# cvxgrp/qcqp

Hardware: AMD Instinct MI355X
Metric: restarts x coord-sweeps / sec (improve COORD_DESCENT phase-2 sweeps, 2n^2 flops each; whole step timed) (higher is better)
Workload: dtype f64

## Files before the change

### qcqp_amd/csrc/cd_life.hip

```cpp
#include "cd_life.h"

#include <cstdio>
#include <cstdlib>

#include "onevar.h"
#include "cd_phase1_sep.h"
#include "cd_chain.h"
#include "cd_roles.h"

namespace qcqpmi {
namespace {

constexpr int L2_WD = 1 << 21;
enum { L2_ABORT = 3 };

__device__ __attribute__((always_inline)) inline RqOwn l2_own(int NB, int CS, int m, int NMW) {
    RqOwn o;
    const int rest = NB - CS;
    o.NB = NB;
    if (m < 0) { o.first = rest; o.stride = 1; o.nu = CS; }
    else { o.first = m; o.stride = NMW; o.nu = m < rest ? (rest - m + NMW - 1) / NMW : 0; }
    return o;
}

constexpr int L2_SHARED_DOUBLES = 8 + 8 + 16 + 8;
constexpr int L2_YBMAX = 18;
constexpr int L2_YU = 6;
constexpr int L2_KCL = 4;
constexpr int l2_tile_doubles(int nmw, int csu, int lr, int kcl = 1, int maxc = 1) {
    return 2 * nmw * 256 + 256 + 256 + 2 * 256 + 2 * 48 + 4 * 256 + csu * 256 + 16 + 8 + 16 * 4 + 8 * 5 + 64 * 10 + 16 * 3 + 8 * 5 + 32 +
           (lr ? L2_YBMAX * 256 + 2 * 256 : 0) +
           2 * (maxc + 1) * 16 * kcl + 2 * 8 * kcl + (kcl > 1 ? 16 : 0);
}
#define L2_LDS_VIEW(tile_) \
    extern __shared__ double smem[]; \
    int *ctl = (int *)smem; \
    int *simdof = (int *)(smem + 8); \
    int *p1cols = (int *)(smem + 16); \
    int *jn = (int *)(smem + 32); \
    double *sp = smem + L2_SHARED_DOUBLES + (tile_) * l2_tile_doubles(NMW, CSU, LRV, KCLV, MAXC); \
    double *part2 = sp; sp += 2 * NMW * 256; \
    double *fixp = sp; sp += 256; \
    double *gtile = sp; sp += 256; \
    double *DU2 = sp; sp += 2 * 256; \
    double *sc2 = sp; sp += 2 * 48; \
    double *ring = sp; sp += 4 * 256; \
    double *cshare = sp; sp += CSU * 256; \
// ... 153 lines not shown
                else L2_LDA(arP + 2 * U, so2 + ((U < nu) ? NMW * 2048 * U : 0), vlane)
            }
        }
        acc = acc + acc1;
        if (i >= 2) {
            const long long tw0 = prof_on ? (long long)__builtin_amdgcn_s_memtime() : 0;
            for (;;) {
                const rq_i4 s4 = rq_sync_read(sy);
                if (s4[RQ_STOP]) { stop = true; break; }
                if (s4[RQ_CONS] >= (int)i - 1) break;
                if (++spins > L2_WD) { stop = true; rq_sync_write(sy, L2_ABORT, 1, lane); rq_sync_write(sy, RQ_STOP, 1, lane); break; }
                __builtin_amdgcn_s_sleep(1);
            }
            if (stop) break;
            spins = 0;
            if (prof_on) pw_cons += (long long)__builtin_amdgcn_s_memtime() - tw0;
        }
        {
            double *part = part2 + (int)(i & 1) * NMW * 256 + m * 256;
    #pragma unroll
            for (int v = 0; v < 4; v++) part[v * 64 + (lane & 15) * 4 + (lane >> 4)] = acc[v];
        }
        rq_sync_write(sy, RQ_PARTS + m, (int)i + 1, lane);
        row = row2;
    }
    if (prof_on && lane == 0) {
        atomicAdd(pprof + 9, (unsigned long long)pw_commit);
        atomicAdd(pprof + 10, (unsigned long long)pw_cons);
    }
    #undef L2_LDA
}


template <int NMW>
__device__ __attribute__((noinline)) void l2_mfma_lr_role(int m_in, int t_in) {
    constexpr int MAXC = 1;
    constexpr int KCLV = 1;
    constexpr int CSU = 1;
    constexpr int LRV = 1;
    constexpr int YU = L2_YU;
    const int tile = l2_uni(t_in);
    L2_LDS_VIEW(tile)
    (void)clsb;
    (void)fixp; (void)gtile; (void)DU2; (void)sc2; (void)cshare; (void)slk; (void)TC; (void)of0; (void)ovis; (void)oacc; (void)oswp; (void)sid; (void)snew;
    (void)sfin; (void)ost; (void)ctl; (void)cst; (void)sseed; (void)sfirst; (void)p1key; (void)p1upd; (void)p1fin; (void)p1sw; (void)p1st; (void)gatep; (void)simdof; (void)p1cols; (void)jn;
    const int lane = threadIdx.x & 63;
    const int m = l2_uni(m_in);
    const double *pG = l2_uni(par->Gpack), *pU = l2_uni(par->Upack);
    const int NB = l2_uni(par->NB), RB = l2_uni(par->RB);
    const int nu = (RB > m) ? (RB - m + NMW - 1) / NMW : 0;
    const int64_t gmax = (int64_t)1 << 40;
    const __amdgpu_buffer_rsrc_t grsrc = __builtin_amdgcn_make_buffer_rsrc(const_cast<double *>(pG), 0, NB * RB * 2048, 0x00020000);
    const __amdgpu_buffer_rsrc_t ursrc = __builtin_amdgcn_make_buffer_rsrc(const_cast<double *>(pU), 0, NB * RB * 2048, 0x00020000);
    const unsigned vlane = (unsigned)lane * 16u;
    typedef unsigned rq_u4 __attribute__((ext_vector_type(4)));
    #define L2_LDF(dst, rs, soff) { const rq_u4 t0_ = __builtin_amdgcn_raw_buffer_load_b128(rs, vlane, (soff), 0);           \
                                    const rq_u4 t1_ = __builtin_amdgcn_raw_buffer_load_b128(rs, vlane + 1024u, (soff), 0);   \
                                    (dst)[0] = __builtin_bit_cast(v2d_, t0_); (dst)[1] = __builtin_bit_cast(v2d_, t1_); }
    typedef __attribute__((address_space(3))) double rq_lds_d;
    typedef __attribute__((address_space(3))) const double rq_lds_cd;
    const int yoff = (lane >> 4) * 16 + (lane & 15);
    rq_lds_d *ybase = (rq_lds_d *)(ytile + yoff);
    rq_lds_cd *rbase = (rq_lds_cd *)(ring + lane);
    rq_lds_cd *pbase = (rq_lds_cd *)(pend + lane);
    asm volatile("" : "+v"(ybase), "+v"(rbase), "+v"(pbase));
    v4d_ y[YU];
    #pragma unroll
    for (int u = 0; u < YU; u++)
    #pragma unroll
        for (int v = 0; v < 4; v++) y[u][v] = (u < nu) ? ybase[(16 * (m + NMW * u) + 4 * v) * 16] : 0.0;
    auto save_y = [&]() {
    #pragma unroll
        for (int u = 0; u < YU; u++)
            if (u < nu) {
    #pragma unroll
                for (int v = 0; v < 4; v++) ybase[(16 * (m + NMW * u) + 4 * v) * 16] = y[u][v];
            }
    };
    int row = 0, spins = 0;
    int yrow = 0;
    int64_t iy = 0;
    for (int64_t i = 0; i < gmax; i++) {
        const int row2 = (row + 1 == NB) ? 0 : row + 1;
        const int ub = row >= 3 ? row - 3 : row - 3 + NB;
        v2d_ aU[YU][2], aG[YU][2];
    #pragma unroll
        for (int u = 0; u < YU; u++)
            if (u < nu) {
                L2_LDF(aU[u], ursrc, (ub * RB + m + NMW * u) * 2048)
                L2_LDF(aG[u], grsrc, (row * RB + m + NMW * u) * 2048)
            }
        bool stop = false;
        if (i >= 3) {
            for (;;) {
                const rq_i4 s4 = rq_sync_read(sy);
                if (s4[RQ_STOP]) { stop = true; break; }
                if (s4[RQ_COMMIT] >= (int)i - 2) break;
                if (++spins > L2_WD) { stop = true; rq_sync_write(sy, L2_ABORT, 1, lane); rq_sync_write(sy, RQ_STOP, 1, lane); break; }
                __builtin_amdgcn_s_sleep(1);
            }
            if (stop) break;
            spins = 0;
        }
        if (i >= 1) {
            if (row == 1) save_y();
            rq_lds_cd *src = (i >= 3) ? rbase + (int)((i - 3) & 3) * 256 : pbase + (int)(i - 1) * 256;
            double bd[4];
    #pragma unroll
            for (int q = 0; q < 4; q++) bd[q] = src[q * 64];
    #pragma unroll
            for (int v = 0; v < 4; v++)
    #pragma unroll
                for (int u = 0; u < YU; u++)
                    if (u < nu) y[u] = __builtin_amdgcn_mfma_f64_16x16x4f64(aU[u][v >> 1][v & 1], bd[v], y[u], 0, 0, 0);
            yrow = row; iy = i;
        }
        v4d_ acc = {0.0, 0.0, 0.0, 0.0}, acc1 = acc;
    #pragma unroll
        for (int u = 0; u < YU; u++)
            if (u < nu) {
                acc = __builtin_amdgcn_mfma_f64_16x16x4f64(aG[u][0][0], y[u][0], acc, 0, 0, 0);
                acc1 = __builtin_amdgcn_mfma_f64_16x16x4f64(aG[u][0][1], y[u][1], acc1, 0, 0, 0);
                acc = __builtin_amdgcn_mfma_f64_16x16x4f64(aG[u][1][0], y[u][2], acc, 0, 0, 0);
                acc1 = __builtin_amdgcn_mfma_f64_16x16x4f64(aG[u][1][1], y[u][3], acc1, 0, 0, 0);
            }
        acc = acc + acc1;
        if (i >= 2) {
            for (;;) {
                const rq_i4 s4 = rq_sync_read(sy);
                if (s4[RQ_STOP]) { stop = true; break; }
                if (s4[RQ_CONS] >= (int)i - 1) break;
                if (++spins > L2_WD) { stop = true; rq_sync_write(sy, L2_ABORT, 1, lane); rq_sync_write(sy, RQ_STOP, 1, lane); break; }
                __builtin_amdgcn_s_sleep(1);
            }
            if (stop) break;
            spins = 0;
        }
        {
            double *part = part2 + (int)(i & 1) * NMW * 256 + m * 256;
    #pragma unroll
            for (int v = 0; v < 4; v++) part[v * 64 + (lane & 15) * 4 + (lane >> 4)] = acc[v];
        }
        rq_sync_write(sy, RQ_PARTS + m, (int)i + 1, lane);
        row = row2;
    }
    if (yrow == NB - 1 && iy >= 3) {
        v2d_ aU[YU][2];
    #pragma unroll
        for (int u = 0; u < YU; u++)
            if (u < nu) L2_LDF(aU[u], ursrc, ((NB - 3) * RB + m + NMW * u) * 2048)
        rq_lds_cd *src = rbase + (int)((iy - 2) & 3) * 256;
        double bd[4];
    #pragma unroll
        for (int q = 0; q < 4; q++) bd[q] = src[q * 64];
    #pragma unroll
        for (int v = 0; v < 4; v++)
    #pragma unroll
            for (int u = 0; u < YU; u++)
                if (u < nu) y[u] = __builtin_amdgcn_mfma_f64_16x16x4f64(aU[u][v >> 1][v & 1], bd[v], y[u], 0, 0, 0);
        save_y();
    } else if (yrow == 0) {
        save_y();
    }
    #undef L2_LDF
}

template <int NMW, int CS, int KIND, int TILES, int LR>
__device__ __attribute__((noinline)) void l2_chain_role(int t_in) {
    constexpr bool MULTI = KIND == L2_KIND_GENK || KIND == L2_KIND_LINK;
    constexpr int BK = KIND == L2_KIND_GENK ? L2_KIND_GEN : KIND == L2_KIND_LINK ? L2_KIND_LIN : KIND;
    constexpr int MAXC = MULTI ? 2 : 1;
    constexpr int KCLV = MULTI ? L2_KCL : 1;
    constexpr int CSU = CS > 0 ? CS : 1;
    constexpr int LRV = LR;
    static_assert(!LR || CS == 0, "factored objective: the chain has no share of the contraction");
    static_assert(!MULTI || (TILES == 1 && !LR), "multi-class kinds: one tile per workgroup, no objective factor");
    constexpr bool PRE = BK == L2_KIND_LIN || BK == L2_KIND_SGN;
    const int tile = TILES > 1 ? l2_uni(t_in) : 0;
    L2_LDS_VIEW(tile)
    (void)ytile; (void)pend; (void)clsb;
    (void)slk; (void)snew; (void)p1key; (void)p1upd; (void)p1fin; (void)p1sw; (void)p1st; (void)gatep; (void)simdof; (void)p1cols; (void)jn;
    const int lane = threadIdx.x & 63, r = lane >> 2, gq = lane & 3;
    GLB const double *Apk = glb(l2_uni(par->Apack));
    GLB const double *Apk2 = glb(l2_uni(par->Apack2));
    GLB const double *Dpk = glb(l2_uni(par->Dpack));
    GLB const double *Spk = glb(l2_uni(par->Spack));
    GLB double *Xg = glb(l2_uni(par->Xg));
    GLB const int *pnext = glb(l2_uni(par->next));
    GLB const int *clsg = glb(l2_uni(par->cls));
    unsigned long long *pprof = l2_uni(par->prof);
    const int pRtotal = l2_uni(par->Rtotal);
    const int NB = l2_uni(par->NB), KS = l2_uni(par->KS), nlast = l2_uni(par->nlast);
    struct { int64_t n; double r0; } P = {(int64_t)l2_uni(par->n), l2_uni(par->r0)};
    struct { double tol, fbound; int64_t num_iters; } a = {l2_uni(par->tol), l2_uni(par->fbound), (int64_t)l2_uni(par->num_iters)};
    const int64_t gmax = (int64_t)1 << 40;
    __builtin_amdgcn_s_setprio(3);
    const int Un = TC.n[r], Uslow = TC.slow[r];
    const double Ul0 = TC.lo[r], Uh0 = TC.hi[r], Ul1 = TC.lo[16 + r], Uh1 = TC.hi[16 + r];
    const bool two = Un >= 2;
    const double thr = two ? 1e-7 * (Ul1 - Uh0) : 0.0;
    const double syma = two ? Ul1 : 0.0, symb = two ? Uh1 : Uh0;
    const double gmid = two ? 0.5 * (Uh0 + Ul1) : QM_INF;
    const double linL = Ul0, linH = two ? Uh1 : Uh0;
    auto lin_tl = [&](double l0_, double h0_, double l1_, double h1_, bool two_) {
        const double lL = l0_, lH = two_ ? h1_ : h0_;
        const double w0 = h0_ - l0_, w1 = two_ ? h1_ - l1_ : w0;
        const double wmin = w0 < w1 ? w0 : w1;
        const double hh = fabs(lL) > fabs(lH) ? fabs(lL) : fabs(lH);
        const double scale = a.fbound * (hh * hh > 1.0 ? hh * hh : 1.0);
        return (wmin > 0.0) ? 0.5e-12 * scale / wmin : QM_INF;
    };
    double tl = 0.0;
    if ((BK == L2_KIND_LIN || BK == L2_KIND_SGN) && !MULTI) tl = lin_tl(Ul0, Uh0, Ul1, Uh1, two);
    const double omid = (BK == L2_KIND_SGN) ? 0.5 * (linL + linH) : 0.0;
    struct { int upd_counter, visits, accepted, sweeps, status; bool conv; } S;
    S.upd_counter = (int)cst[0 * 64 + lane]; S.visits = (int)cst[1 * 64 + lane]; S.accepted = (int)cst[2 * 64 + lane];
    S.sweeps = (int)cst[3 * 64 + lane]; S.conv = cst[4 * 64 + lane] != 0; S.status = (int)cst[5 * 64 + lane];
    double fpart = __longlong_as_double(cst[6 * 64 + lane]);
    bool frz = (cst[7 * 64 + lane] & 1) != 0, done = (cst[7 * 64 + lane] & 2) != 0, pre = PRE && (cst[7 * 64 + lane] & 4) != 0;
    bool ld = LR && (cst[7 * 64 + lane] & 8) != 0;
    double facc = __longlong_as_double(cst[8 * 64 + lane]);
    const bool occupied = sid[r] >= 0;
    const RqOwn cown = l2_own(NB, CS, -1, NMW);
    v2d_ arC[2 * CSU];
    double afix[4] = {0.0, 0.0, 0.0, 0.0}, afix2[4] = {0.0, 0.0, 0.0, 0.0};
    v4d_ carry = {0.0, 0.0, 0.0, 0.0};
    double xon[4], d4[4], s3 = 0.0;
    {
    #pragma unroll
        for (int e = 0; e < 4; e++) d4[e] = Dpk[lane + 64 * e];
        if (lane < 48) s3 = Spk[lane];
    #pragma unroll
        for (int v = 0; v < 4; v++) xon[v] = Xg[(4 * v + gq) * 16 + r];
    #pragma unroll
        for (int e = 0; e < 4; e++) DU2[lane + 64 * e] = d4[e];
        if (lane < 48) sc2[lane] = s3;
        if (MULTI && lane < 16) clsb[lane] = (lane < l2_uni(par->n)) ? clsg[lane] : 0;
        v4d_ c0 = {0.0, 0.0, 0.0, 0.0}, c1 = {0.0, 0.0, 0.0, 0.0};
        const int bl2 = NB - 2, bl1 = NB - 1;
        double f0a[4], f0b[4], f1b[4], x2[4], x1[4];
    #pragma unroll
        for (int u = 0; u < 4; u++) {
            f0a[u] = Apk[((int64_t)0 * KS + 4 * bl2 + u) * 64 + lane];
            f0b[u] = Apk[((int64_t)0 * KS + 4 * bl1 + u) * 64 + lane];
            f1b[u] = Apk[((int64_t)1 * KS + 4 * bl1 + u) * 64 + lane];
            x2[u] = LR ? pend[u * 64 + lane] : Xg[(4 * bl2 + u) * 64 + lane];
            x1[u] = LR ? pend[256 + u * 64 + lane] : Xg[(4 * bl1 + u) * 64 + lane];
        }
    #pragma unroll
        for (int u = 0; u < 4; u++) c0 = __builtin_amdgcn_mfma_f64_16x16x4f64(f0a[u], x2[u], c0, 0, 0, 0);
    #pragma unroll
        for (int u = 0; u < 4; u++) {
            c0 = __builtin_amdgcn_mfma_f64_16x16x4f64(f0b[u], x1[u], c0, 0, 0, 0);
            c1 = __builtin_amdgcn_mfma_f64_16x16x4f64(f1b[u], x1[u], c1, 0, 0, 0);
        }
        carry = c1;
        if (CS > 0) {
            rq_load_A<CSU>(arC, Apk2, KS, cown, lane, 0);
            double bqC[4 * CSU];
    #pragma unroll
            for (int U = 0; U < CSU; U++) {
                const int bb = rq_block(cown, U);
    #pragma unroll
                for (int q = 0; q < 4; q++) bqC[4 * U + q] = Xg[(4 * bb + q) * 64 + lane];
            }
    #pragma unroll
            for (int U = 0; U < CSU; U++)
    #pragma unroll
                for (int q = 0; q < 4; q++) cshare[U * 256 + q * 64 + lane] = bqC[4 * U + q];
            c0 = rq_product<CSU>(arC, bqC, Apk2, KS, cown, lane, rq_slot(cown, bl1), rq_slot(cown, bl2), 1, c0);
        }
    #pragma unroll
        for (int v = 0; v < 4; v++) fixp[v * 64 + (lane & 15) * 4 + (lane >> 4)] = c0[v];
    }
    const double tolv = a.tol;
    int b = 0, spins = 0;
    bool wdog = false;
    const bool prof_on = pprof != nullptr;
    long long pw_part = 0, pt_sum = 0, pt_steps = 0, pt_end = 0, pt_fix = 0, pt_req = 0, ptl = 0;
    if (prof_on) { ptl = (long long)__builtin_amdgcn_s_memtime(); if (lane == 0) atomicAdd(pprof + 18, (unsigned long long)(ptl - *(long long *)(ctl + 6))); }
    int pn_int = 0, pn_gen = 0;
#define L2_TICK(acc) if (prof_on) { const long long now_ = (long long)__builtin_amdgcn_s_memtime(); acc += now_ - ptl; ptl = now_; }
    int64_t last_g = 0;
    for (int64_t g = 0; g < gmax; g++) {
        last_g = g;
        const int bn = (b + 1 == NB) ? 0 : b + 1, bn2 = (bn + 1 == NB) ? 0 : bn + 1;
        const int bprev = (b == 0) ? NB - 1 : b - 1;
        const int cur = (int)(g & 1);
        const double *DU = DU2 + cur * 256, *hqb = sc2 + cur * 48, *rtb = sc2 + cur * 48 + 16, *dgb = sc2 + cur * 48 + 32;
        const double *part = part2 + cur * NMW * 256;
        double *rb = ring + (int)(g & 3) * 256;
        const int ncol = (b == NB - 1) ? nlast : 16;
        double xo[4];
    #pragma unroll
        for (int v = 0; v < 4; v++) xo[v] = xon[v];
    #pragma unroll
        for (int e = 0; e < 4; e++) d4[e] = Dpk[(int64_t)bn * 256 + lane + 64 * e];
        if (lane < 48) s3 = Spk[(int64_t)bn * 48 + lane];
        int c3 = 0;
        if (MULTI && lane < 16) c3 = (16 * bn + lane < (int)P.n) ? clsg[16 * bn + lane] : 0;
    #pragma unroll
        for (int v = 0; v < 4; v++) xon[v] = Xg[(16 * (int64_t)bn + 4 * v + gq) * 16 + r];
        {
            GLB const double *ap = Apk + ((int64_t)bn * KS + 4 * b) * 64 + lane;
            GLB const double *ap2 = Apk + ((int64_t)bn2 * KS + 4 * b) * 64 + lane;
    #pragma unroll
            for (int u = 0; u < 4; u++) { afix[u] = ap[u * 64]; afix2[u] = ap2[u * 64]; }
        }
        const long long tw0 = prof_on ? (long long)__builtin_amdgcn_s_memtime() : 0;
        for (;;) {
            const rq_i4 p4 = rq_sync_read(sy + RQ_PARTS);
            int lo4 = p4[0] < p4[1] ? p4[0] : p4[1];
            const int lo2 = p4[2] < p4[3] ? p4[2] : p4[3];
            lo4 = lo4 < lo2 ? lo4 : lo2;
            if (NMW > 4) {
                const rq_i4 q4 = rq_sync_read(sy + RQ_PARTS + 4);
                const int l1 = q4[0] < q4[1] ? q4[0] : q4[1], l2 = q4[2] < q4[3] ? q4[2] : q4[3];
                lo4 = lo4 < l1 ? lo4 : l1;
                lo4 = lo4 < l2 ? lo4 : l2;
            }
            if (lo4 >= (int)g + 1) break;
            if (++spins > L2_WD) { wdog = true; break; }
            __builtin_amdgcn_s_sleep(1);
        }
        if (wdog) { rq_sync_write(sy, L2_ABORT, 1, lane); break; }
        spins = 0;
        if (prof_on) { pt_req += tw0 - ptl; ptl = (long long)__builtin_amdgcn_s_memtime(); pw_part += ptl - tw0; pn_int++; }
        double gb[4], xn[4], rto[4], t2o[4], hq4[4];
    #pragma unroll
        for (int v = 0; v < 4; v++) {
            double s = fixp[v * 64 + lane];
    #pragma unroll
            for (int w = 0; w < NMW; w++) s += part[w * 256 + v * 64 + lane];
            hq4[v] = hqb[4 * v + gq];
            s += hq4[v];
            gb[v] = s;
            gtile[(4 * v + gq) * 16 + r] = s;
        }
        rq_sync_write(sy, RQ_CONS, (int)g + 1, lane);
    #pragma unroll
// ... 167 lines not shown
                    DrawKey dk{dseed, dfirst + (uint64_t)sid[r], (uint32_t)i, (uint32_t)(G.sweeps - 1) | 0x80000000u, 0u};
                    double xnew = xi;
                    int got;
                    if (BK == L2_KIND_LIN && cslow == 0 && C.n > 0 && fabs(gc) > ctl_) {
                        xnew = (gc > 0.0) ? clinL : clinH;
                        got = G.conv ? 0 : 1;
                    } else {
                        got = G.conv ? 0 : onevar_minimise<MAXC>(t2g, t1, t0, C, dk, &xnew);
                    }
                    bool moved;
                    double delta;
                    const bool wasconv = G.conv;
                    chain_commit<MAXC>(G, got, xnew, xi, t2g, t1, t0, a.tol, P.n, moved, delta);
                    if (!wasconv) fa = moved ? 0.0 : fa + xi * (gc + hq);
                    if (moved) {
                        rb[c * 16 + r] = xnew;
                        for (int c2 = c + 1; c2 < 16; c2++) gtile[c2 * 16 + r] += DU[c * 16 + c2] * delta;
                    }
                }
                S.upd_counter = (int)G.upd_counter; S.visits = (int)G.visits; S.accepted = (int)G.accepted; S.conv = G.conv; S.status = G.status;
                fpart = (gq == 0) ? G.fcur : 0.0;
                facc = (gq == 0) ? fa : 0.0;
                if (S.conv) done = true;
#pragma unroll
                for (int v = 0; v < 4; v++) xn[v] = rb[(4 * v + gq) * 16 + r];
                if (LR) {
#pragma unroll
                    for (int v = 0; v < 4; v++) rb[(4 * v + gq) * 16 + r] = xn[v] - xo[v];
                }
            }
        }
    #pragma unroll
        for (int v = 0; v < 4; v++) Xg[(16 * (int64_t)b + 4 * v + gq) * 16 + r] = xn[v];
        rq_sync_write(sy, RQ_COMMIT, (int)g + 1, lane);
        L2_TICK(pt_end)
        if (b == NB - 1) {
            if (ld) { ld = false; if (!frz) S.conv = false; }
            else if (frz) { frz = false; done = true; }
            if (PRE && pre) {
                const double f0s = rq_quad_sum(facc) + P.r0;
                fpart = (gq == 0) ? f0s : 0.0;
                facc = 0.0; pre = false; S.conv = false;
            }
        }
        const unsigned long long livem = __builtin_amdgcn_ballot_w64(!S.conv || frz || pre || ld);
        if (TILES == 1) {
            if (livem == 0ull) break;
            if (b == NB - 1) {
                const bool fin = !occupied || done;
                const unsigned long long finm = __builtin_amdgcn_ballot_w64(fin);
                if (finm == ~0ull) break;
                if (finm != 0ull) {
                    const bool more = glb_load_int(pnext) < pRtotal;
                    if (more) break;
                }
            }
        } else if (b == NB - 1) {
            const unsigned long long finm = __builtin_amdgcn_ballot_w64(!occupied || done);
            const int mine = (livem != 0ull ? 1 : 0) | (finm == ~0ull ? 2 : 0) | (finm != 0ull ? 4 : 0);
            const int tag = ((int)(g / NB) + 1) << 8;
            rq_lds_int *jw = (rq_lds_int *)jn;
            int verdict = 0;
            if (tile == 1) rq_sync_write(jw, 1, tag | mine, lane);
            for (;;) {
                int w = *(volatile rq_lds_int *)(jw + (tile == 1 ? 0 : 1));
                asm volatile("" ::: "memory");
                w = __builtin_amdgcn_readfirstlane(w);
                if ((w & ~0xff) == tag) { verdict = w & 0xff; break; }
                if (++spins > L2_WD) { wdog = true; break; }
                __builtin_amdgcn_s_sleep(1);
            }
            if (wdog) { rq_sync_write(sy, L2_ABORT, 1, lane); break; }
            spins = 0;
            if (tile == 0) {
                const int both = mine | verdict, all = mine & verdict;
                bool stop = !(both & 1) || (all & 2);
                if (!stop && (both & 4)) stop = glb_load_int(pnext) < pRtotal;
                rq_sync_write(jw, 0, tag | (stop ? 1 : 0), lane);
                verdict = stop ? 1 : 0;
            }
            if (verdict & 1) break;
        }
        {
            v4d_ acc = carry, acc2 = {0.0, 0.0, 0.0, 0.0};
            double xb4[4];
    #pragma unroll
            for (int u = 0; u < 4; u++) xb4[u] = rb[u * 64 + lane];
    #pragma unroll
            for (int u = 0; u < 4; u++) {
                acc = __builtin_amdgcn_mfma_f64_16x16x4f64(afix[u], xb4[u], acc, 0, 0, 0);
                acc2 = __builtin_amdgcn_mfma_f64_16x16x4f64(afix2[u], xb4[u], acc2, 0, 0, 0);
            }
            carry = acc2;
            if (CS > 0) {
                const int us = rq_slot(cown, b);
                if (us >= 0) {
    #pragma unroll
                    for (int q = 0; q < 4; q++) cshare[us * 256 + q * 64 + lane] = xb4[q];
                }
                double bqC[4 * CSU];
    #pragma unroll
                for (int U = 0; U < CSU; U++)
    #pragma unroll
                    for (int q = 0; q < 4; q++) bqC[4 * U + q] = cshare[U * 256 + q * 64 + lane];
                acc = rq_product<CSU>(arC, bqC, Apk2, KS, cown, lane, us, rq_slot(cown, bprev), bn2, acc);
            }
    #pragma unroll
            for (int v = 0; v < 4; v++) fixp[v * 64 + (lane & 15) * 4 + (lane >> 4)] = acc[v];
        }
        {
            const int nx = (int)((g + 1) & 1);
    #pragma unroll
            for (int e = 0; e < 4; e++) DU2[nx * 256 + lane + 64 * e] = d4[e];
            if (lane < 48) sc2[nx * 48 + lane] = s3;
            if (MULTI && lane < 16) clsb[nx * 16 + lane] = c3;
        }
        L2_TICK(pt_fix)
        b = bn;
    }
#undef L2_TICK
    if (LR) {
        const int g1 = (int)((last_g - 1) & 3), g0 = (int)(last_g & 3);
        double p1v[4], p0v[4];
#pragma unroll
        for (int u = 0; u < 4; u++) { p1v[u] = ring[g1 * 256 + u * 64 + lane]; p0v[u] = ring[g0 * 256 + u * 64 + lane]; }
#pragma unroll
        for (int u = 0; u < 4; u++) { pend[u * 64 + lane] = p1v[u]; pend[256 + u * 64 + lane] = p0v[u]; }
    }
    rq_sync_write(sy, RQ_STOP, 1, lane);
    if (prof_on && lane == 0) {
        atomicAdd(pprof + 13, (unsigned long long)pt_sum);
        atomicAdd(pprof + 14, (unsigned long long)pt_steps);
        atomicAdd(pprof + 15, (unsigned long long)pt_end);
        atomicAdd(pprof + 19, (unsigned long long)pt_req);
        *(long long *)(ctl + 8) = (long long)__builtin_amdgcn_s_memtime();
        atomicAdd(pprof + 7, (unsigned long long)pt_fix);
        atomicAdd(pprof + 8, (unsigned long long)pw_part);
        atomicAdd(pprof + 11, (unsigned long long)pn_int);
        atomicAdd(pprof + 12, (unsigned long long)pn_gen);
    }
    {
        cst[0 * 64 + lane] = S.upd_counter; cst[1 * 64 + lane] = S.visits; cst[2 * 64 + lane] = S.accepted;
        cst[3 * 64 + lane] = S.sweeps; cst[4 * 64 + lane] = S.conv ? 1 : 0; cst[5 * 64 + lane] = S.status;
        cst[6 * 64 + lane] = __double_as_longlong(fpart);
        cst[7 * 64 + lane] = (frz ? 1 : 0) | (done ? 2 : 0) | (pre ? 4 : 0) | (ld ? 8 : 0);
        cst[8 * 64 + lane] = __double_as_longlong(facc);
        const double ftot = rq_quad_sum(facc) + P.r0;
        const bool fin = occupied && done;
        if (gq == 0) {
            sfin[r] = fin ? 1 : 0;
            if (fin) { ovis[r] = S.visits; oacc[r] = S.accepted; oswp[r] = S.sweeps; ost[r] = S.status; of0[r] = ftot; }
        }
    }
    __builtin_amdgcn_s_setprio(0);
}

template <int NMW, int CS, int KIND, int TILES, int LR>
__global__ __launch_bounds__((NMW == 3 && TILES == 1) ? 256 : 512, 2) void cd_life_kernel(CdLife2Args a0) {
    const CdLife2Args &a = a0;
    constexpr bool MULTI = KIND == L2_KIND_GENK || KIND == L2_KIND_LINK;
    constexpr int BK = KIND == L2_KIND_GENK ? L2_KIND_GEN : KIND == L2_KIND_LINK ? L2_KIND_LIN : KIND;
    constexpr int MAXC = MULTI ? 2 : 1;
    constexpr int KCLV = MULTI ? L2_KCL : 1;
    constexpr int CSU = CS > 0 ? CS : 1;
    constexpr int LRV = LR;
    static_assert(!MULTI || (TILES == 1 && !LR), "multi-class kinds: one tile per workgroup, no objective factor");
    constexpr int NT = (NMW == 3 && TILES == 1) ? 256 : 512;
    constexpr int NW = NT / 64;
    constexpr int NS = 16 * TILES;
    constexpr int TD = l2_tile_doubles(NMW, CSU, LR);
    static_assert(!LR || (NMW == 3 && CS == 0 && BK != L2_KIND_LIN && BK != L2_KIND_SGN), "factored objective: three multiplying waves per tile, no chain share, a positive diagonal");
    constexpr bool PRE = BK == L2_KIND_LIN || BK == L2_KIND_SGN;
    static_assert(TILES == 1 || NMW == 3, "two tiles per workgroup: eight waves = two chains + two x three multiplying waves");
    const DevProblem &P = a.P;
    const int tid0 = threadIdx.x;
    const int wave = __builtin_amdgcn_readfirstlane(tid0 >> 6);
    const int64_t n16 = P.n16;
    const int NB = (int)P.NB, KS = (int)P.KS;
    L2_LDS_VIEW(0)
    (void)fixp; (void)gtile; (void)DU2; (void)sc2; (void)ring; (void)cshare; (void)of0; (void)ovis; (void)oacc; (void)oswp; (void)ost; (void)ytile; (void)pend; (void)clsb;
#define L2_STORE_SETS(st_, sc_, slack_) {                                                                                              \
        SetTable<MAXC> T2 = TC;                                                                                                          \
        T2.lo = l2_tl(TC.lo, st_, TD); T2.hi = l2_tl(TC.hi, st_, TD); T2.n = l2_tl(TC.n, st_, TD); T2.slow = l2_tl(TC.slow, st_, TD);    \
        const int nk_ = MULTI ? a0.nclass : 1;                                                                                           \
        for (int k_ = 0; k_ < nk_; k_++) {                                                                                               \
            FeasSet<MAXC> C_;                                                                                                            \
            compute_set<MAXC>(P, P.krep[k_], slack_, C_);                                                                                \
            store_set<MAXC>(T2, 16 * k_ + (sc_), C_);                                                                                    \
            if (MULTI && C_.n > 2) T2.slow[16 * k_ + (sc_)] = 1;                                                                         \
        }                                                                                                                                \
    }
    GLB double *Xg0 = glb(a0.scratch) + (int64_t)blockIdx.x * TILES * n16 * 16;

    if ((tid0 & 63) == 0) simdof[wave] = (int)(__builtin_amdgcn_s_getreg(4 | (4 << 6) | (1 << 11)));
    if (NMW == 3 && TILES == 1 && tid0 == 0) {
        int arrival = 0;
        if (a0.cuslot) {
            const unsigned hw = __builtin_amdgcn_s_getreg(4 | (0 << 6) | (31 << 11)), xcc = __builtin_amdgcn_s_getreg(20 | (0 << 6) | (31 << 11));
            arrival = glb_add(glb(a0.cuslot) + (((xcc & 15) << 8) | (((hw >> 12) & 15) << 4) | ((hw >> 8) & 15)), 1);
        }
        simdof[8] = (arrival & 1) ? (a0.rotmode == 2 ? 16 + 1 : 2) : 0;
    }
    if (tid0 < 64 * TILES) {
// ... 45 lines not shown
        pr->NB = NB; pr->KS = KS; pr->n = (int)P.n; pr->nlast = nlast; pr->Rtotal = (int)lf0->Rtotal; pr->dbg = a0.dbg;
        pr->cls = P.cls;
    }
    __syncthreads();

    for (;;) {
        int tid = tid0;
        asm volatile("" : "+v"(tid));
        const CdLife *lifep = a0.life;
        asm volatile("" : "+s"(lifep));
        const int lane = tid & 63, r = lane >> 2;
        if (tid == 0) { ctl[0] = 0; jn[0] = 0; jn[1] = 0; }
        __syncthreads();
        if (tid < NS) {
            const int st = tid >> 4, sc = tid & 15;
            int id = l2_tl(sid, st, TD)[sc], nw = 0;
            if (id < 0) {
                GLB const CdLife *lf = glb(lifep);
                const int idx = glb_add(glb(a0.b.next), 1);
                if (idx < (int)lf->Rtotal) {
                    id = idx; nw = 1;
                    const uint64_t pop = (uint64_t)idx / (uint64_t)lf->Rpop, rho = (uint64_t)idx % (uint64_t)lf->Rpop;
                    l2_tl(sseed, st, TD)[sc] = lf->seed + pop * lf->seed_stride;
                    l2_tl(sfirst, st, TD)[sc] = lf->first_index + pop * lf->first_stride + rho - (uint64_t)idx;
                }
            }
            l2_tl(sid, st, TD)[sc] = id; l2_tl(snew, st, TD)[sc] = nw;
            if (nw) { l2_tl(p1fin, st, TD)[sc] = 0; l2_tl(p1sw, st, TD)[sc] = 0; l2_tl(p1st, st, TD)[sc] = 0; l2_tl(gatep, st, TD)[sc] = 0; }
            if (id < 0) {
                l2_tl(slk, st, TD)[sc] = 0.0;
                L2_STORE_SETS(st, sc, 0.0)
            }
            if (id >= 0) atomicAdd(&ctl[0], 1);
            *(volatile rq_lds_int *)(l2_tl((int *)sy, st, TD) + sc) = (sc >= RQ_PARTS + NMW) ? 0x7fffffff : 0;
        }
        __syncthreads();
        if (ctl[0] == 0) break;
        {
            __builtin_amdgcn_s_setprio(3);
            GLB const CdLife *lf = glb(lifep);
            const long long pt0 = lf->prof ? (long long)__builtin_amdgcn_s_memtime() : 0;
            const int lf_pre = LR ? lf->prebuilt : 0;
            const int lf_generate = lf->generate && !lf_pre, lf_phase1 = lf->phase1 && !lf_pre;
            const double lf_viol_tol = lf->viol_tol;
            const int e0 = P.cptr[P.krep[0]];
            const double cp = P.cp[e0], cq = P.cq[e0], cr = P.cr[e0];
            const int rel = P.crel[e0];
            for (int c = 0; c < NS; c++) {
                const int ct = c >> 4, cc = c & 15;
                GLB double *Xg = Xg0 + (int64_t)ct * n16 * 16;
                if (!l2_tl(snew, ct, TD)[cc]) {
                    if (l2_tl(sid, ct, TD)[cc] < 0) for (int64_t j = tid; j < n16; j += NT) Xg[j * 16 + cc] = 0.0;
                    continue;
                }
                if (!lf_generate) {
                    const int id = l2_tl(sid, ct, TD)[cc];
                    GLB const double *src = glb(a0.b.X) + ((int64_t)(id >> 4) * n16) * 16 + (id & 15);
                    for (int64_t j0 = tid; j0 < n16; j0 += 4 * NT) {
                        double t4[4];
#pragma unroll
                        for (int u = 0; u < 4; u++) t4[u] = (j0 + u * NT < n16) ? src[(j0 + u * NT) * 16] : 0.0;
#pragma unroll
                        for (int u = 0; u < 4; u++) if (j0 + u * NT < n16) Xg[(j0 + u * NT) * 16 + cc] = t4[u];
                    }
                }
            }
            if (lf_generate) {
// ... 158 lines not shown
                        else l2_tl(ytile, ct, TD)[(rowz - 32) * 16 + cc] = 0.0;
                    }
                }
                __syncthreads();
            }
            if (lf->prof && tid == 0) {
                int nn = 0;
                for (int k = 0; k < NS; k++) nn += l2_tl(snew, k >> 4, TD)[k & 15] ? 1 : 0;
                atomicAdd((unsigned long long *)lf->prof + 0, (unsigned long long)((long long)__builtin_amdgcn_s_memtime() - pt0));
                atomicAdd((unsigned long long *)lf->prof + 2, 1ull);
                atomicAdd((unsigned long long *)lf->prof + 3, (unsigned long long)nn);
            }
            __builtin_amdgcn_s_setprio(0);
        }
        if (role == 0) {
            long long *cs_ = l2_tl(cst, rtile, TD);
            if (l2_tl(snew, rtile, TD)[r]) {
#pragma unroll
                for (int f = 0; f < 6; f++) cs_[f * 64 + lane] = 0;
                const int pass = l2_tl(gatep, rtile, TD)[r];
                cs_[6 * 64 + lane] = 0;
                cs_[4 * 64 + lane] = (pass && !PRE && !LR) ? 0 : 1;
                cs_[7 * 64 + lane] = (pass ? (PRE ? 4 : 0) : 1) | (LR ? 8 : 0);
                cs_[8 * 64 + lane] = 0;
            } else if (l2_tl(sid, rtile, TD)[r] < 0) {
                cs_[4 * 64 + lane] = 1; cs_[6 * 64 + lane] = 0;
                cs_[7 * 64 + lane] = 2; cs_[8 * 64 + lane] = 0;
            }
        }
        __syncthreads();
        if (tid == 0 && glb(lifep)->prof) *(long long *)(ctl + 6) = (long long)__builtin_amdgcn_s_memtime();

        if (role > 0) {
            if (LR) l2_mfma_lr_role<NMW>(role - 1, rtile);
            else l2_mfma_role<NMW, CS>(role - 1, rtile);
        } else l2_chain_role<NMW, CS, KIND, TILES, LR>(rtile);

        __syncthreads();
        if (sy[L2_ABORT] || (TILES > 1 && l2_tl((int *)sy, 1, TD)[L2_ABORT])) {
            if (tid == 0) __hip_atomic_store(glb(a0.abort), 1, __ATOMIC_RELAXED, __HIP_MEMORY_SCOPE_AGENT);
            break;
        }
        if (tid == 0 && glb(lifep)->prof)
        {
            const long long now_ = (long long)__builtin_amdgcn_s_memtime();
            atomicAdd((unsigned long long *)glb(lifep)->prof + 5, (unsigned long long)(now_ - *(long long *)(ctl + 6)));
            atomicAdd((unsigned long long *)glb(lifep)->prof + 20, (unsigned long long)(now_ - *(long long *)(ctl + 8)));
        }
        {
            const int e0 = P.cptr[P.krep[0]];
            const double cp = P.cp[e0], cq = P.cq[e0], cr = P.cr[e0];
            const int rel = P.crel[e0];
            if (tid == 0) { int cnt = 0; for (int k = 0; k < NS; k++) if (l2_tl(sfin, k >> 4, TD)[k & 15]) p1cols[cnt++] = k; ctl[4] = cnt; }
            if (tid < NS) l2_tl(p1key, tid >> 4, TD)[tid & 15] = ordered_key(-QM_INF);
            __syncthreads();
            const int nfin = ctl[4];
            const int64_t items = (int64_t)nfin * n16;
            for (int64_t w0 = tid; w0 < items; w0 += (int64_t)NT * 8) {
                double xv8[8];
#pragma unroll
                for (int u = 0; u < 8; u++) {
                    const int64_t w = w0 + (int64_t)NT * u;
                    const int col = p1cols[w < items ? w / n16 : 0];
                    const int64_t i = w % n16;
                    xv8[u] = (w < items && i < P.n) ? (Xg0 + (int64_t)(col >> 4) * n16 * 16)[i * 16 + (col & 15)] : 0.0;
                }
#pragma unroll
// ... 237 lines not shown
}

int cd_life2_tiles(const DevProblem &P, int nmw, int cs, int64_t restarts, int cus, int requested, int lr) {
    (void)P; (void)restarts; (void)cus;
    if (!lr || nmw != 3 || cs != 0) return 1;
    int t = requested;
    if (const char *ev = getenv("QCQPMI_L2_TILES")) t = atoi(ev);
    return t == 2 ? 2 : 1;
}

int cd_life2_pack(const DevProblem &P, double *Dpack, double *Spack, hipStream_t st) {
    hipLaunchKernelGGL(l2_pack_kernel, dim3((unsigned)P.NB), dim3(256), 0, st, P, Dpack, Spack);
    return (int)hipGetLastError();
}

int cd_life2_launch(const CdLife2Args &a, int nmw, int cs, int kind, int tiles, int wgs, hipStream_t st) {
    const int lr = a.RB > 0 ? 1 : 0;
    if (const char *ev = getenv("QCQPMI_L2_CS")) {
        const int k2 = atoi(ev);
        if (!lr && nmw == 3 && tiles == 1 && (k2 == 0 || k2 == 2 || k2 == 4) && k2 + 3 <= (int)a.P.NB && (int)a.P.NB - k2 <= 3 * RQ_MAXU) cs = k2;
    }
    const size_t lds = cd_life2_lds_bytes(nmw, cs, tiles, lr, kind);
    if (getenv("QCQPMI_L2_DEBUG")) {
        int occ = -1;
        hipError_t e = lr ? (tiles == 2 ? hipOccupancyMaxActiveBlocksPerMultiprocessor(&occ, cd_life_kernel<3, 0, L2_KIND_BAND, 2, 1>, 512, lds)
                                        : hipOccupancyMaxActiveBlocksPerMultiprocessor(&occ, cd_life_kernel<3, 0, L2_KIND_BAND, 1, 1>, 256, lds))
                     : nmw == 3 ? hipOccupancyMaxActiveBlocksPerMultiprocessor(&occ, cd_life_kernel<3, 4, L2_KIND_BAND, 1, 0>, 256, lds)
                                : hipOccupancyMaxActiveBlocksPerMultiprocessor(&occ, cd_life_kernel<7, 4, L2_KIND_BAND, 1, 0>, 512, lds);
        fprintf(stderr, "cd_life2_launch: nmw %d cs %d kind %d tiles %d lr %d wgs %d lds %zu: occupancy %d workgroups per CU (%s)\n", nmw, cs, kind, tiles, lr, wgs, lds, occ, hipGetErrorString(e));
    }
    if (wgs < 1) wgs = 1;
    if (lr) {
        if (nmw != 3 || cs != 0 || kind == L2_KIND_LIN || kind == L2_KIND_SGN) return (int)hipErrorInvalidValue;
        return tiles == 2 ? l2_launch_kind<3, 0, 2, 1>(a, kind, wgs, lds, st) : l2_launch_kind<3, 0, 1, 1>(a, kind, wgs, lds, st);
    }
    if (tiles != 1) return (int)hipErrorInvalidValue;
    if (nmw == 3) {
        if (cs == 0) return l2_launch_kind<3, 0, 1, 0>(a, kind, wgs, lds, st);
        if (cs == 2) return l2_launch_kind<3, 2, 1, 0>(a, kind, wgs, lds, st);
        if (cs == 4) return l2_launch_kind<3, 4, 1, 0>(a, kind, wgs, lds, st);
        return (int)hipErrorInvalidValue;
    }
    if (nmw == 7 && cs == 4) return l2_launch_kind<7, 4, 1, 0>(a, kind, wgs, lds, st);
    return (int)hipErrorInvalidValue;
}

const char *cd_life2_name(int nmw, int kind, int tiles, int lr) {
    if (kind == L2_KIND_GENK) return nmw == 3 ? "cd_life_kernel<3,gen,classes>" : "cd_life_kernel<7,gen,classes>";
    if (kind == L2_KIND_LINK) return nmw == 3 ? "cd_life_kernel<3,lin,classes>" : "cd_life_kernel<7,lin,classes>";
    if (kind == L2_KIND_SGN) return nmw == 3 ? "cd_life_kernel<3,sgn>" : "cd_life_kernel<7,sgn>";
    if (lr) return tiles == 2 ? (kind == L2_KIND_BAND ? "cd_life_kernel<3,band,2 tiles,factored>" : "cd_life_kernel<3,gen,2 tiles,factored>")
                              : (kind == L2_KIND_BAND ? "cd_life_kernel<3,band,factored>" : "cd_life_kernel<3,gen,factored>");
    if (tiles == 2) return kind == L2_KIND_BAND ? "cd_life_kernel<3,band,2 tiles>" : kind == L2_KIND_GEN ? "cd_life_kernel<3,gen,2 tiles>" : "cd_life_kernel<3,lin,2 tiles>";
    if (nmw == 3) return kind == L2_KIND_BAND ? "cd_life_kernel<3,band>" : kind == L2_KIND_GEN ? "cd_life_kernel<3,gen>" : "cd_life_kernel<3,lin>";
    return kind == L2_KIND_BAND ? "cd_life_kernel<7,band>" : kind == L2_KIND_GEN ? "cd_life_kernel<7,gen>" : "cd_life_kernel<7,lin>";
}

}
```

Before: 28.00 million.

## Offload chain-wave carry product and D/S prefetch to last multiplying wave

```diff
diff --git a/qcqp_amd/csrc/cd_life.hip b/qcqp_amd/csrc/cd_life.hip
--- a/qcqp_amd/csrc/cd_life.hip
+++ b/qcqp_amd/csrc/cd_life.hip
@@ -13,6 +13,11 @@
 
 constexpr int L2_WD = 1 << 21;
 enum { L2_ABORT = 3 };
+enum { L2_AUXW = 12 };
+enum { L2_LR_NONE = 0, L2_LR_AUX = 1, L2_LR_CHAIN = 2 };
+#ifndef L2_AUX_PARTS
+#define L2_AUX_PARTS 3
+#endif
 
 __device__ __attribute__((always_inline)) inline RqOwn l2_own(int NB, int CS, int m, int NMW) {
     RqOwn o;
@@ -232,7 +237,7 @@
 }
 
 
-template <int NMW>
+template <int NMW, int AUX>
 __device__ __attribute__((noinline)) void l2_mfma_lr_role(int m_in, int t_in) {
     constexpr int MAXC = 1;
     constexpr int KCLV = 1;
@@ -249,6 +254,15 @@
     const double *pG = l2_uni(par->Gpack), *pU = l2_uni(par->Upack);
     const int NB = l2_uni(par->NB), RB = l2_uni(par->RB);
     const int nu = (RB > m) ? (RB - m + NMW - 1) / NMW : 0;
+    const bool auxw = AUX && m == NMW - 1;
+    constexpr bool AUXC = AUX != 0 && (L2_AUX_PARTS & 1) != 0, AUXS = AUX != 0 && (L2_AUX_PARTS & 2) != 0;
+    GLB const double *Apk = glb(l2_uni(par->Apack));
+    GLB const double *Dpk = glb(l2_uni(par->Dpack));
+    GLB const double *Spk = glb(l2_uni(par->Spack));
+    const int KS = l2_uni(par->KS);
+    unsigned long long *pprof = l2_uni(par->prof);
+    const bool prof_on = AUX && pprof != nullptr;
+    long long pt_aux = 0;
     const int64_t gmax = (int64_t)1 << 40;
     const __amdgpu_buffer_rsrc_t grsrc = __builtin_amdgcn_make_buffer_rsrc(const_cast<double *>(pG), 0, NB * RB * 2048, 0x00020000);
     const __amdgpu_buffer_rsrc_t ursrc = __builtin_amdgcn_make_buffer_rsrc(const_cast<double *>(pU), 0, NB * RB * 2048, 0x00020000);
@@ -290,6 +304,20 @@
                 L2_LDF(aU[u], ursrc, (ub * RB + m + NMW * u) * 2048)
                 L2_LDF(aG[u], grsrc, (row * RB + m + NMW * u) * 2048)
             }
+        const int rowp = row == 0 ? NB - 1 : row - 1;
+        double aA[4] = {0.0, 0.0, 0.0, 0.0}, dS[4] = {0.0, 0.0, 0.0, 0.0}, sS = 0.0;
+        if (AUX && auxw && i >= 3) {
+            GLB const double *ap = Apk + ((int64_t)rowp * KS + 4 * ub) * 64 + lane;
+            if (AUXC) {
+    #pragma unroll
+                for (int u = 0; u < 4; u++) aA[u] = ap[u * 64];
+            }
+            if (AUXS) {
+    #pragma unroll
+                for (int e = 0; e < 4; e++) dS[e] = Dpk[(int64_t)rowp * 256 + lane + 64 * e];
+                if (lane < 48) sS = Spk[(int64_t)rowp * 48 + lane];
+            }
+        }
         bool stop = false;
         if (i >= 3) {
             for (;;) {
@@ -303,11 +331,29 @@
             spins = 0;
         }
         if (i >= 1) {
-            if (row == 1) save_y();
             rq_lds_cd *src = (i >= 3) ? rbase + (int)((i - 3) & 3) * 256 : pbase + (int)(i - 1) * 256;
             double bd[4];
     #pragma unroll
             for (int q = 0; q < 4; q++) bd[q] = src[q * 64];
+            if (AUX && auxw && i >= 3) {
+                const long long ta0 = prof_on ? (long long)__builtin_amdgcn_s_memtime() : 0;
+                if (AUXC) {
+                    v4d_ cz = {0.0, 0.0, 0.0, 0.0};
+    #pragma unroll
+                    for (int u = 0; u < 4; u++) cz = __builtin_amdgcn_mfma_f64_16x16x4f64(aA[u], bd[u], cz, 0, 0, 0);
+    #pragma unroll
+                    for (int v = 0; v < 4; v++) cshare[v * 64 + lane] = cz[v];
+                }
+                if (AUXS) {
+                    const int nx = (int)((i - 1) & 1);
+    #pragma unroll
+                    for (int e = 0; e < 4; e++) DU2[nx * 256 + lane + 64 * e] = dS[e];
+                    if (lane < 48) sc2[nx * 48 + lane] = sS;
+                }
+                rq_sync_write(sy, L2_AUXW, (int)i - 1, lane);
+                if (prof_on) pt_aux += (long long)__builtin_amdgcn_s_memtime() - ta0;
+            }
+            if (row == 1) save_y();
     #pragma unroll
             for (int v = 0; v < 4; v++)
     #pragma unroll
@@ -362,6 +408,7 @@
     } else if (yrow == 0) {
         save_y();
     }
+    if (prof_on && auxw && lane == 0) atomicAdd(pprof + 23, (unsigned long long)pt_aux);
     #undef L2_LDF
 }
 
@@ -372,7 +419,9 @@
     constexpr int MAXC = MULTI ? 2 : 1;
     constexpr int KCLV = MULTI ? L2_KCL : 1;
     constexpr int CSU = CS > 0 ? CS : 1;
-    constexpr int LRV = LR;
+    constexpr int LRV = LR ? 1 : 0;
+    constexpr bool AUX = LR == L2_LR_AUX;
+    constexpr bool AUXC = AUX != 0 && (L2_AUX_PARTS & 1) != 0, AUXS = AUX != 0 && (L2_AUX_PARTS & 2) != 0;
     static_assert(!LR || CS == 0, "factored objective: the chain has no share of the contraction");
     static_assert(!MULTI || (TILES == 1 && !LR), "multi-class kinds: one tile per workgroup, no objective factor");
     constexpr bool PRE = BK == L2_KIND_LIN || BK == L2_KIND_SGN;
@@ -435,6 +484,14 @@
     #pragma unroll
         for (int e = 0; e < 4; e++) DU2[lane + 64 * e] = d4[e];
         if (lane < 48) sc2[lane] = s3;
+        if (AUXS) {
+    #pragma unroll
+            for (int e = 0; e < 4; e++) d4[e] = Dpk[256 + lane + 64 * e];
+            if (lane < 48) s3 = Spk[48 + lane];
+    #pragma unroll
+            for (int e = 0; e < 4; e++) DU2[256 + lane + 64 * e] = d4[e];
+            if (lane < 48) sc2[48 + lane] = s3;
+        }
         if (MULTI && lane < 16) clsb[lane] = (lane < l2_uni(par->n)) ? clsg[lane] : 0;
         v4d_ c0 = {0.0, 0.0, 0.0, 0.0}, c1 = {0.0, 0.0, 0.0, 0.0};
         const int bl2 = NB - 2, bl1 = NB - 1;
@@ -455,6 +512,10 @@
             c1 = __builtin_amdgcn_mfma_f64_16x16x4f64(f1b[u], x1[u], c1, 0, 0, 0);
         }
         carry = c1;
+        if (AUXC) {
+    #pragma unroll
+            for (int v = 0; v < 4; v++) cshare[v * 64 + lane] = c1[v];
+        }
         if (CS > 0) {
             rq_load_A<CSU>(arC, Apk2, KS, cown, lane, 0);
             double bqC[4 * CSU];
@@ -477,7 +538,7 @@
     int b = 0, spins = 0;
     bool wdog = false;
     const bool prof_on = pprof != nullptr;
-    long long pw_part = 0, pt_sum = 0, pt_steps = 0, pt_end = 0, pt_fix = 0, pt_req = 0, ptl = 0;
+    long long pw_part = 0, pw_aux = 0, pt_sum = 0, pt_steps = 0, pt_end = 0, pt_fix = 0, pt_req = 0, ptl = 0;
     if (prof_on) { ptl = (long long)__builtin_amdgcn_s_memtime(); if (lane == 0) atomicAdd(pprof + 18, (unsigned long long)(ptl - *(long long *)(ctl + 6))); }
     int pn_int = 0, pn_gen = 0;
 #define L2_TICK(acc) if (prof_on) { const long long now_ = (long long)__builtin_amdgcn_s_memtime(); acc += now_ - ptl; ptl = now_; }
@@ -494,9 +555,11 @@
         double xo[4];
     #pragma unroll
         for (int v = 0; v < 4; v++) xo[v] = xon[v];
-    #pragma unroll
-        for (int e = 0; e < 4; e++) d4[e] = Dpk[(int64_t)bn * 256 + lane + 64 * e];
-        if (lane < 48) s3 = Spk[(int64_t)bn * 48 + lane];
+        if (!AUXS) {
+    #pragma unroll
+            for (int e = 0; e < 4; e++) d4[e] = Dpk[(int64_t)bn * 256 + lane + 64 * e];
+            if (lane < 48) s3 = Spk[(int64_t)bn * 48 + lane];
+        }
         int c3 = 0;
         if (MULTI && lane < 16) c3 = (16 * bn + lane < (int)P.n) ? clsg[16 * bn + lane] : 0;
     #pragma unroll
@@ -505,7 +568,7 @@
             GLB const double *ap = Apk + ((int64_t)bn * KS + 4 * b) * 64 + lane;
             GLB const double *ap2 = Apk + ((int64_t)bn2 * KS + 4 * b) * 64 + lane;
     #pragma unroll
-            for (int u = 0; u < 4; u++) { afix[u] = ap[u * 64]; afix2[u] = ap2[u * 64]; }
+            for (int u = 0; u < 4; u++) { afix[u] = ap[u * 64]; if (!AUXC) afix2[u] = ap2[u * 64]; }
         }
         const long long tw0 = prof_on ? (long long)__builtin_amdgcn_s_memtime() : 0;
         for (;;) {
@@ -739,6 +802,26 @@
         }
     #pragma unroll
         for (int v = 0; v < 4; v++) Xg[(16 * (int64_t)b + 4 * v + gq) * 16 + r] = xn[v];
+        if (AUX) {
+            if (g >= 1) {
+                const long long tw0 = prof_on ? (long long)__builtin_amdgcn_s_memtime() : 0;
+                for (;;) {
+                    const rq_i4 s4 = rq_sync_read(sy);
+                    const rq_i4 a4 = rq_sync_read(sy + L2_AUXW);
+                    if (s4[RQ_STOP]) { wdog = true; break; }
+                    if (a4[0] >= (int)g + 1) break;
+                    if (++spins > L2_WD) { wdog = true; break; }
+                    __builtin_amdgcn_s_sleep(1);
+                }
+                if (wdog) { rq_sync_write(sy, L2_ABORT, 1, lane); break; }
+                spins = 0;
+                if (prof_on) { const long long w_ = (long long)__builtin_amdgcn_s_memtime() - tw0; pw_aux += w_; ptl += w_; }
+            }
+            if (AUXC) {
+    #pragma unroll
+                for (int v = 0; v < 4; v++) carry[v] = cshare[v * 64 + lane];
+            }
+        }
         rq_sync_write(sy, RQ_COMMIT, (int)g + 1, lane);
         L2_TICK(pt_end)
         if (b == NB - 1) {
@@ -796,9 +879,9 @@
     #pragma unroll
             for (int u = 0; u < 4; u++) {
                 acc = __builtin_amdgcn_mfma_f64_16x16x4f64(afix[u], xb4[u], acc, 0, 0, 0);
-                acc2 = __builtin_amdgcn_mfma_f64_16x16x4f64(afix2[u], xb4[u], acc2, 0, 0, 0);
-            }
-            carry = acc2;
+                if (!AUXC) acc2 = __builtin_amdgcn_mfma_f64_16x16x4f64(afix2[u], xb4[u], acc2, 0, 0, 0);
+            }
+            if (!AUXC) carry = acc2;
             if (CS > 0) {
                 const int us = rq_slot(cown, b);
                 if (us >= 0) {
@@ -815,7 +898,7 @@
     #pragma unroll
             for (int v = 0; v < 4; v++) fixp[v * 64 + (lane & 15) * 4 + (lane >> 4)] = acc[v];
         }
-        {
+        if (!AUXS) {
             const int nx = (int)((g + 1) & 1);
     #pragma unroll
             for (int e = 0; e < 4; e++) DU2[nx * 256 + lane + 64 * e] = d4[e];
@@ -845,6 +928,7 @@
         atomicAdd(pprof + 8, (unsigned long long)pw_part);
         atomicAdd(pprof + 11, (unsigned long long)pn_int);
         atomicAdd(pprof + 12, (unsigned long long)pn_gen);
+        if (AUX) atomicAdd(pprof + 22, (unsigned long long)pw_aux);
     }
     {
         cst[0 * 64 + lane] = S.upd_counter; cst[1 * 64 + lane] = S.visits; cst[2 * 64 + lane] = S.accepted;
@@ -870,12 +954,13 @@
     constexpr int MAXC = MULTI ? 2 : 1;
     constexpr int KCLV = MULTI ? L2_KCL : 1;
     constexpr int CSU = CS > 0 ? CS : 1;
-    constexpr int LRV = LR;
+    constexpr int LRV = LR ? 1 : 0;
+    constexpr int AUX = LR == L2_LR_AUX ? 1 : 0;
     static_assert(!MULTI || (TILES == 1 && !LR), "multi-class kinds: one tile per workgroup, no objective factor");
     constexpr int NT = (NMW == 3 && TILES == 1) ? 256 : 512;
     constexpr int NW = NT / 64;
     constexpr int NS = 16 * TILES;
-    constexpr int TD = l2_tile_doubles(NMW, CSU, LR);
+    constexpr int TD = l2_tile_doubles(NMW, CSU, LRV);
     static_assert(!LR || (NMW == 3 && CS == 0 && BK != L2_KIND_LIN && BK != L2_KIND_SGN), "factored objective: three multiplying waves per tile, no chain share, a positive diagonal");
     constexpr bool PRE = BK == L2_KIND_LIN || BK == L2_KIND_SGN;
     static_assert(TILES == 1 || NMW == 3, "two tiles per workgroup: eight waves = two chains + two x three multiplying waves");
@@ -987,7 +1072,7 @@
                 L2_STORE_SETS(st, sc, 0.0)
             }
             if (id >= 0) atomicAdd(&ctl[0], 1);
-            *(volatile rq_lds_int *)(l2_tl((int *)sy, st, TD) + sc) = (sc >= RQ_PARTS + NMW) ? 0x7fffffff : 0;
+            *(volatile rq_lds_int *)(l2_tl((int *)sy, st, TD) + sc) = (sc >= RQ_PARTS + NMW && !(AUX && sc == L2_AUXW)) ? 0x7fffffff : 0;
         }
         __syncthreads();
         if (ctl[0] == 0) break;
@@ -1212,7 +1297,7 @@
         if (tid == 0 && glb(lifep)->prof) *(long long *)(ctl + 6) = (long long)__builtin_amdgcn_s_memtime();
 
         if (role > 0) {
-            if (LR) l2_mfma_lr_role<NMW>(role - 1, rtile);
+            if (LR) l2_mfma_lr_role<NMW, AUX>(role - 1, rtile);
             else l2_mfma_role<NMW, CS>(role - 1, rtile);
         } else l2_chain_role<NMW, CS, KIND, TILES, LR>(rtile);
 
@@ -1516,7 +1601,10 @@
     if (wgs < 1) wgs = 1;
     if (lr) {
         if (nmw != 3 || cs != 0 || kind == L2_KIND_LIN || kind == L2_KIND_SGN) return (int)hipErrorInvalidValue;
-        return tiles == 2 ? l2_launch_kind<3, 0, 2, 1>(a, kind, wgs, lds, st) : l2_launch_kind<3, 0, 1, 1>(a, kind, wgs, lds, st);
+        const char *aux_ev = getenv("QCQPMI_L2_AUX");
+        if (aux_ev && atoi(aux_ev) == 0)
+            return tiles == 2 ? l2_launch_kind<3, 0, 2, L2_LR_CHAIN>(a, kind, wgs, lds, st) : l2_launch_kind<3, 0, 1, L2_LR_CHAIN>(a, kind, wgs, lds, st);
+        return tiles == 2 ? l2_launch_kind<3, 0, 2, L2_LR_AUX>(a, kind, wgs, lds, st) : l2_launch_kind<3, 0, 1, L2_LR_AUX>(a, kind, wgs, lds, st);
     }
     if (tiles != 1) return (int)hipErrorInvalidValue;
     if (nmw == 3) {
```

New measurement: 27.06 million. 0.966x the previous value.
